# ubuntuslave/vo_single_camera_sos

Measured on AMD Instinct MI355X. Metric: frame-pairs/sec (detect+match+triangulate+RANSAC) on 640x480 omni, 2000 kpts, higher is better.
Workload: dtype u8/f32/f64

## Files before the change

include/sosvo.h:

```cpp
#ifndef SOSVO_H
#define SOSVO_H

#include <stdint.h>

#ifdef __cplusplus
extern "C" {
#endif

typedef struct sosvo_ctx sosvo_ctx;

typedef enum {
  SOSVO_OK = 0,
  SOSVO_ERR_ARG = -1,
  SOSVO_ERR_HIP = -2,
  SOSVO_ERR_NODEVICE = -3,
  SOSVO_ERR_CAPACITY = -4
} sosvo_status;

#define SOSVO_DESC_BYTES 32
#define SOSVO_KEY_SHIFT 20
#define SOSVO_KEY_IDX_MASK 0xFFFFFu
#define SOSVO_KEY_NONE 0xFFFFFFFFu


int32_t sosvo_abi_version(void);

int32_t sosvo_orb_bit_pattern_31(int8_t* pattern_host);

int32_t sosvo_create(sosvo_ctx** out, int32_t device, void* stream);
int32_t sosvo_destroy(sosvo_ctx* ctx);
int32_t sosvo_set_stream(sosvo_ctx* ctx, void* stream);
#define SOSVO_HINT_SHARED_DEVICE 1
#define SOSVO_HINT_SCORE_FP64_ONLY 2
int32_t sosvo_set_hint(sosvo_ctx* ctx, int32_t hint, int32_t value);
int32_t sosvo_synchronize(sosvo_ctx* ctx);
const char* sosvo_last_error(const sosvo_ctx* ctx);

int32_t sosvo_timer_start(sosvo_ctx* ctx);
int32_t sosvo_timer_stop(sosvo_ctx* ctx);
int32_t sosvo_timer_elapsed_ms(sosvo_ctx* ctx, float* ms);

int32_t sosvo_profile_enable(sosvo_ctx* ctx, int32_t on);
int32_t sosvo_profile_count(sosvo_ctx* ctx);
int32_t sosvo_profile_get(sosvo_ctx* ctx, int32_t i, char* name_out, int32_t name_cap, float* ms);

int32_t sosvo_debug_fill_scratch(sosvo_ctx* ctx, int32_t byte);

int32_t sosvo_unwrap(sosvo_ctx* ctx, const uint8_t* omni, const uint8_t* masks, const float* map_x,
                     const float* map_y, int32_t nframes, int32_t H, int32_t W, int32_t rows,
                     int32_t cols, uint8_t* pano);

int32_t sosvo_unwrap_prepare(sosvo_ctx* ctx, const uint8_t* masks, const float* map_x, const float* map_y,
                             int32_t H, int32_t W, int32_t rows, int32_t cols, uint32_t* table);
int32_t sosvo_unwrap_table(sosvo_ctx* ctx, const uint8_t* omni, const uint32_t* table, int32_t nframes,
                           int32_t H, int32_t W, int32_t rows, int32_t cols, uint8_t* pano);

int32_t sosvo_median_gray(sosvo_ctx* ctx, const uint8_t* img, int32_t nimg, int32_t rows,
                          int32_t cols, int32_t ksize, uint8_t* gray);
int32_t sosvo_unwrap_median_gray(sosvo_ctx* ctx, const uint8_t* omni, const uint32_t* table, int32_t nframes,
                                 int32_t H, int32_t W, int32_t rows, int32_t cols, int32_t ksize, uint8_t* gray);

int32_t sosvo_unwrap_median_gray_rows(sosvo_ctx* ctx, const uint8_t* omni, const uint32_t* table, int32_t nframes,
                                      int32_t H, int32_t W, int32_t rows, int32_t cols, int32_t ksize,
                                      const int32_t* row_range, uint8_t* gray);

int32_t sosvo_gray_rows_needed(sosvo_ctx* ctx, const uint32_t* mask_bits, int32_t nsets, int32_t rows, int32_t cols,
                               int32_t nmask, int32_t edge, const int8_t* pattern, float cos_a, float sin_a,
                               int32_t* row_range);

int32_t sosvo_detect_gft(sosvo_ctx* ctx, const uint8_t* gray, const uint32_t* mask_bits, int32_t nimg,
                         int32_t images_per_maskset, int32_t rows, int32_t cols, int32_t nmask,
                         double quality, double min_distance, int32_t max_corners, int32_t cap,
                         float* kp, int32_t* n, int32_t* status);

int32_t sosvo_describe_orb(sosvo_ctx* ctx, const uint8_t* gray, int32_t nimg, int32_t rows, int32_t cols,
                           int32_t nmask, int32_t cap, float* kp, int32_t* n, float cos_a, float sin_a,
                           const int8_t* pattern, int32_t edge, uint8_t* desc);

int32_t sosvo_describe_orb_rows(sosvo_ctx* ctx, const uint8_t* gray, int32_t nimg, int32_t rows, int32_t cols,
                                int32_t nmask, int32_t cap, float* kp, int32_t* n, float cos_a, float sin_a,
                                const int8_t* pattern, int32_t edge, const int32_t* row_range, uint8_t* desc);

int64_t sosvo_orb_pyramid_pixels(int32_t rows, int32_t cols);
int32_t sosvo_orb_mask_pyramid(sosvo_ctx* ctx, const uint32_t* mask_bits, int32_t nsets, int32_t rows,
                               int32_t cols, int32_t nmask, uint32_t* mask_pyr);
int32_t sosvo_detect_orb(sosvo_ctx* ctx, const uint8_t* gray, const uint32_t* mask_pyr, int32_t nimg,
                         int32_t images_per_maskset, int32_t rows, int32_t cols, int32_t nmask,
                         int32_t nfeatures, int32_t cap, float* kp4, float* resp, int32_t* n);
int32_t sosvo_describe_orb_levels(sosvo_ctx* ctx, const uint8_t* gray, int32_t nimg, int32_t rows,
                                  int32_t cols, int32_t nmask, int32_t cap, float* kp4, int32_t* n,
                                  const int8_t* pattern, uint8_t* desc, float* kp_xy);
int32_t sosvo_detect_describe_orb(sosvo_ctx* ctx, const uint8_t* gray, const uint32_t* mask_pyr, int32_t nimg,
                                  int32_t images_per_maskset, int32_t rows, int32_t cols, int32_t nmask,
                                  int32_t nfeatures, int32_t cap, float* kp4, float* resp, int32_t* n,
                                  const int8_t* pattern, uint8_t* desc, float* kp_xy);

int32_t sosvo_detect_fast(sosvo_ctx* ctx, const uint8_t* gray, const uint32_t* mask_bits, int32_t nimg,
                          int32_t images_per_maskset, int32_t rows, int32_t cols, int32_t nmask,
                          int32_t threshold, int32_t cap, float* kp, int32_t* n, int32_t* status);

int32_t sosvo_detect_agast(sosvo_ctx* ctx, const uint8_t* gray, const uint32_t* mask_bits, int32_t nimg,
                           int32_t images_per_maskset, int32_t rows, int32_t cols, int32_t nmask,
                           int32_t threshold, int32_t cap, float* kp, int32_t* n, int32_t* status);

int32_t sosvo_match_hamming(sosvo_ctx* ctx, const uint8_t* q_desc, const uint8_t* t_desc,
                            const int32_t* nq, const int32_t* nt, const int32_t* q_slot,
                            const int32_t* t_slot, int32_t nprob, int32_t q_stride,
                            int32_t t_stride, int32_t k, uint32_t* keys);

int32_t sosvo_match_hamming_gated(sosvo_ctx* ctx, const uint8_t* q_desc, const uint8_t* t_desc, const float* q_pos,
                                  const float* t_pos, const int32_t* nq, const int32_t* nt, const int32_t* q_slot,
                                  const int32_t* t_slot, int32_t nprob, int32_t n_forward, int32_t q_stride, int32_t t_stride,
                                  double min_dv, double max_du, int32_t max_distance, uint32_t* keys);

// ... 246 lines not shown
```

vo_single_camera_sos_amd/_lib.py:

```python
import ctypes
import os
import re

_HERE = os.path.dirname(os.path.abspath(__file__))
LIB_PATH = os.path.join(_HERE, "libsosvo.so")
HEADER_PATH = os.path.join(os.path.dirname(_HERE), "include", "sosvo.h")

c_i32 = ctypes.c_int32
c_f64 = ctypes.c_double
c_f32 = ctypes.c_float
c_u64 = ctypes.c_uint64
c_p = ctypes.c_void_p

SOSVO_OK = 0
STATUS_NAMES = {0: "SOSVO_OK", -1: "SOSVO_ERR_ARG", -2: "SOSVO_ERR_HIP", -3: "SOSVO_ERR_NODEVICE",
                -4: "SOSVO_ERR_CAPACITY"}

KEY_SHIFT = 20
KEY_IDX_MASK = 0xFFFFF
KEY_NONE = 0xFFFFFFFF
DESC_BYTES = 32


class SosvoError(RuntimeError):
    pass


SIGNATURES = {
    "sosvo_abi_version": (c_i32, []),
    "sosvo_orb_bit_pattern_31": (c_i32, [c_p]),
    "sosvo_create": (c_i32, [ctypes.POINTER(c_p), c_i32, c_p]),
    "sosvo_destroy": (c_i32, [c_p]),
    "sosvo_set_stream": (c_i32, [c_p, c_p]),
    "sosvo_set_hint": (c_i32, [c_p, c_i32, c_i32]),
    "sosvo_synchronize": (c_i32, [c_p]),
    "sosvo_last_error": (ctypes.c_char_p, [c_p]),
    "sosvo_timer_start": (c_i32, [c_p]),
    "sosvo_timer_stop": (c_i32, [c_p]),
    "sosvo_timer_elapsed_ms": (c_i32, [c_p, ctypes.POINTER(c_f32)]),
    "sosvo_profile_enable": (c_i32, [c_p, c_i32]),
    "sosvo_profile_count": (c_i32, [c_p]),
    "sosvo_debug_fill_scratch": (c_i32, [c_p, c_i32]),
    "sosvo_profile_get": (c_i32, [c_p, c_i32, ctypes.c_char_p, c_i32, ctypes.POINTER(c_f32)]),
    "sosvo_unwrap": (c_i32, [c_p, c_p, c_p, c_p, c_p, c_i32, c_i32, c_i32, c_i32, c_i32, c_p]),
    "sosvo_unwrap_prepare": (c_i32, [c_p, c_p, c_p, c_p, c_i32, c_i32, c_i32, c_i32, c_p]),
    "sosvo_unwrap_table": (c_i32, [c_p, c_p, c_p, c_i32, c_i32, c_i32, c_i32, c_i32, c_p]),
    "sosvo_median_gray": (c_i32, [c_p, c_p, c_i32, c_i32, c_i32, c_i32, c_p]),
    "sosvo_unwrap_median_gray": (c_i32, [c_p, c_p, c_p, c_i32, c_i32, c_i32, c_i32, c_i32, c_i32, c_p]),
    "sosvo_unwrap_median_gray_rows": (c_i32, [c_p, c_p, c_p, c_i32, c_i32, c_i32, c_i32, c_i32, c_i32, c_p, c_p]),
    "sosvo_gray_rows_needed": (c_i32, [c_p, c_p, c_i32, c_i32, c_i32, c_i32, c_i32, c_p, c_f32, c_f32, c_p]),
    "sosvo_detect_gft": (c_i32, [c_p, c_p, c_p, c_i32, c_i32, c_i32, c_i32, c_i32, c_f64, c_f64, c_i32, c_i32, c_p,
                                 c_p, c_p]),
    "sosvo_describe_orb": (c_i32, [c_p, c_p, c_i32, c_i32, c_i32, c_i32, c_i32, c_p, c_p, c_f32, c_f32, c_p, c_i32,
                                   c_p]),
    "sosvo_describe_orb_rows": (c_i32, [c_p, c_p, c_i32, c_i32, c_i32, c_i32, c_i32, c_p, c_p, c_f32, c_f32, c_p, c_i32,
                                        c_p, c_p]),
    "sosvo_orb_pyramid_pixels": (ctypes.c_int64, [c_i32, c_i32]),
    "sosvo_orb_mask_pyramid": (c_i32, [c_p, c_p, c_i32, c_i32, c_i32, c_i32, c_p]),
    "sosvo_detect_orb": (c_i32, [c_p, c_p, c_p, c_i32, c_i32, c_i32, c_i32, c_i32, c_i32, c_i32, c_p, c_p, c_p]),
    "sosvo_describe_orb_levels": (c_i32, [c_p, c_p, c_i32, c_i32, c_i32, c_i32, c_i32, c_p, c_p, c_p, c_p, c_p]),
    "sosvo_detect_describe_orb": (c_i32, [c_p, c_p, c_p, c_i32, c_i32, c_i32, c_i32, c_i32, c_i32, c_i32, c_p, c_p, c_p, c_p,
                                          c_p, c_p]),
    "sosvo_detect_fast": (c_i32, [c_p, c_p, c_p, c_i32, c_i32, c_i32, c_i32, c_i32, c_i32, c_i32, c_p, c_p, c_p]),
    "sosvo_detect_agast": (c_i32, [c_p, c_p, c_p, c_i32, c_i32, c_i32, c_i32, c_i32, c_i32, c_i32, c_p, c_p, c_p]),
    "sosvo_match_hamming": (c_i32, [c_p, c_p, c_p, c_p, c_p, c_p, c_p, c_i32, c_i32, c_i32, c_i32, c_p]),
    "sosvo_match_hamming_gated": (c_i32, [c_p, c_p, c_p, c_p, c_p, c_p, c_p, c_p, c_p, c_i32, c_i32, c_i32, c_i32, c_f64, c_f64,
                                          c_i32, c_p]),
    "sosvo_match_radius": (c_i32, [c_p, c_p, c_p, c_p, c_p, c_p, c_p, c_i32, c_i32, c_i32, c_i32, c_i32, c_p, c_p]),
    "sosvo_cross_check_matches": (c_i32, [c_p, c_p, c_p, c_p, c_p, c_p, c_p, c_i32, c_i32, c_i32, c_p, c_p]),
    "sosvo_sort_matches": (c_i32, [c_p, c_p, c_p, c_p, c_i32, c_i32, c_p]),
    "sosvo_pano_to_bearing": (c_i32, [c_p, c_p, c_i32, c_f64, c_f64, c_f64, c_f64, c_p, c_p, c_p]),
    "sosvo_triangulate_midpoint": (c_i32, [c_p, c_p, c_p, c_p, c_p, c_i32, c_p, c_p, c_p]),
    "sosvo_triangulate2": (c_i32, [c_p, c_p, c_p, c_i32, c_p, c_p, c_p]),
    "sosvo_range_filter": (c_i32, [c_p, c_p, c_i32, c_f64, c_f64, c_p]),
    "sosvo_rgbd_backproject": (c_i32, [c_p, c_p, c_i32, c_i32, c_p, c_p, c_i32, c_f64, c_f64, c_f64, c_f64, c_f64,
                                       c_i32, c_p, c_p]),
    "sosvo_stereo_assemble": (c_i32, [c_p] + [c_p] * 9 + [c_i32] * 4 + [c_p] * 9),
    "sosvo_f2f_assemble": (c_i32, [c_p] + [c_p] * 7 + [c_i32] + [c_p] * 6 + [c_i32, c_i32] + [c_p] * 7),
    "sosvo_ransac_abs_pose": (c_i32, [c_p, c_p, c_p, c_p, c_p, c_p, c_i32, c_i32, c_p, c_i32, c_i32, c_f64,
                                      c_i32, c_i32, c_u64, c_p, c_p, c_p, c_p, c_p, c_p]),
    "sosvo_ransac_abs_pose_seeds": (c_i32, [c_p, c_p, c_p, c_p, c_p, c_p, c_i32, c_i32, c_p, c_i32, c_i32, c_f64,
                                            c_i32, c_i32, c_p, c_p, c_p, c_p, c_p, c_p, c_p]),
    "sosvo_match_l2": (c_i32, [c_p, c_p, c_p, c_p, c_p, c_i32, c_i32, c_i32, c_i32, c_i32, c_p]),
    "sosvo_ransac_rel_pose": (c_i32, [c_p, c_p, c_p, c_p, c_i32, c_i32, c_i32, c_f64, c_i32, c_i32, c_u64, c_p, c_p, c_p, c_p,
                                      c_p, c_p]),
    "sosvo_refine_abs_pose": (c_i32, [c_p, c_p, c_p, c_p, c_p, c_p, c_i32, c_p, c_i32, c_i32, c_p, c_p, c_i32,
                                      c_p, c_p, c_p]),
    "sosvo_rgbd_assemble": (c_i32, [c_p, c_p, c_p, c_p, c_p, c_p, c_i32, c_i32, c_i32, c_i32, c_i32, c_p, c_p, c_p, c_p, c_p]),
    "sosvo_f2f_assemble_central": (c_i32, [c_p, c_f64, c_f64, c_p, c_p, c_p, c_p, c_i32, c_p, c_p, c_p, c_p, c_i32, c_i32,
                                           c_p, c_p, c_p, c_p, c_p]),
    "sosvo_frame_pair_batch_workspace": (ctypes.c_size_t, [c_p]),
    "sosvo_frame_pair_batch": (c_i32, [c_p, c_p, c_p, c_p, c_p, c_p, c_p, c_p, ctypes.c_size_t, c_p]),
    "sosvo_frame_pair_batch_streams_workspace": (ctypes.c_size_t, [c_p, c_i32]),
    "sosvo_frame_pair_batch_streams": (c_i32, [c_p, c_p, c_p, c_i32, c_p, c_p, c_p, c_p, c_p, ctypes.c_size_t, c_p]),
    "sosvo_frame_pair_batch_streams_enqueue": (c_i32, [c_p, c_p, c_p, c_i32, c_p, c_p, c_p, c_p, c_p, ctypes.c_size_t, c_p]),
    "sosvo_frame_pair_batch_streams_join": (c_i32, [c_p]),
    "sosvo_sequence_workspace": (ctypes.c_size_t, [c_p, c_i32, c_i32]),
    "sosvo_sequence_front_end": (c_i32, [c_p, c_p, c_p, c_i32, c_i32, c_p, c_i32, c_i32, c_p, c_p, c_p, c_p, ctypes.c_size_t]),
    "sosvo_sequence_track": (c_i32, [c_p, c_p, c_p, c_i32, c_i32, c_p, c_p, c_i32, c_u64, c_p, ctypes.c_size_t, c_p]),
    "sosvo_sequence_copy_slot": (c_i32, [c_p, c_p, c_i32, c_i32, c_i32, c_i32, c_p, ctypes.c_size_t]),
    "sosvo_sequence_frame_counts": (c_i32, [c_p, c_p, c_i32, c_i32, c_i32, c_i32, c_p, ctypes.c_size_t, c_p]),
    "sosvo_sequence_front_end_slots": (c_i32, [c_p, c_p, c_p, c_i32, c_i32, c_p, c_i32, c_p, c_p, c_p, c_p, c_p, ctypes.c_size_t]),
    "sosvo_sequence_track_seeds": (c_i32, [c_p, c_p, c_p, c_i32, c_i32, c_p, c_p, c_p, c_i32, c_p, ctypes.c_size_t, c_p]),
    "sosvo_sequence_copy_slots": (c_i32, [c_p, c_p, c_i32, c_i32, c_p, c_p, c_i32, c_p, ctypes.c_size_t]),
    "sosvo_rgbd_sequence_workspace": (ctypes.c_size_t, [c_p, c_i32, c_i32]),
    "sosvo_rgbd_sequence_front_end": (c_i32, [c_p, c_p, c_p, c_i32, c_i32, c_p, c_p, c_i32, c_i32, c_p, c_p, c_p, ctypes.c_size_t]),
    "sosvo_rgbd_sequence_track": (c_i32, [c_p, c_p, c_i32, c_i32, c_p, c_p, c_i32, c_u64, c_p, ctypes.c_size_t, c_p]),
    "sosvo_rgbd_sequence_copy_slot": (c_i32, [c_p, c_p, c_i32, c_i32, c_i32, c_i32, c_p, ctypes.c_size_t]),
    "sosvo_rgbd_sequence_frame_counts": (c_i32, [c_p, c_p, c_i32, c_i32, c_i32, c_i32, c_p, ctypes.c_size_t, c_p]),
    "sosvo_rgbd_sequence_front_end_slots": (c_i32, [c_p, c_p, c_p, c_i32, c_i32, c_p, c_p, c_i32, c_p, c_p, c_p, c_p,
                                                    ctypes.c_size_t]),
    "sosvo_rgbd_sequence_track_seeds": (c_i32, [c_p, c_p, c_i32, c_i32, c_p, c_p, c_p, c_i32, c_p, ctypes.c_size_t, c_p]),
    "sosvo_rgbd_sequence_copy_slots": (c_i32, [c_p, c_p, c_i32, c_i32, c_p, c_p, c_i32, c_p, ctypes.c_size_t]),
    "sosvo_rgbd_pair_batch_workspace": (ctypes.c_size_t, [c_p]),
    "sosvo_rgbd_pair_batch": (c_i32, [c_p, c_p, c_p, c_p, c_p, c_p, c_p, c_p, ctypes.c_size_t, c_p]),
}

HINT_SHARED_DEVICE = 1
HINT_SCORE_FP64_ONLY = 2
FLAG_CAM_ROT_IDENTITY = 1
FLAG_EPNP = 2
FLAG_GP3P = 4
FLAG_TWOPT = 8
FLAG_CROSS_CHECK_STEREO = 0x1000
FLAG_CROSS_CHECK_F2F = 0x2000
FLAG_GATED_STEREO = 0x4000
FLAG_GATED_F2F = 0x8000
GATED_MAX_DIST_SHIFT = 16
GATED_MAX_DIST_MASK = 0x1FF << GATED_MAX_DIST_SHIFT
DETECTOR_GFT = 0
DETECTOR_ORB = 1
DETECTOR_FAST = 2
DETECTOR_AGAST = 3
DETECTORS = {"GFT": DETECTOR_GFT, "ORB": DETECTOR_ORB, "FAST": DETECTOR_FAST, "AGAST": DETECTOR_AGAST}
RGBD_DETECTOR_SHIFT = 8
RGBD_DETECTOR_MASK = 3 << RGBD_DETECTOR_SHIFT
REL_FIVEPT = 5
REL_SEVENPT = 7
REL_EIGHTPT = 8


class Rig(ctypes.Structure):
    _fields_ = [("pano_top", c_f64 * 4), ("pano_bot", c_f64 * 4), ("F_top", c_f64 * 3), ("F_bot", c_f64 * 3),
                ("min_range", c_f64), ("max_range", c_f64), ("stereo_min_disp", c_f64),
                ("stereo_max_hdiff", c_f64), ("f2f_max_hdiff", c_f64), ("pct_good_matches", c_f64)]



class RgbdCam(ctypes.Structure):
    _fields_ = [("fx", c_f64), ("fy", c_f64), ("cx", c_f64), ("cy", c_f64), ("focal_length_m", c_f64),
                ("depth_is_Z", c_i32), ("reserved", c_i32), ("min_range", c_f64), ("max_range", c_f64)]

# ... 74 lines not shown
```

vo_single_camera_sos_amd/csrc/common.h:

```cpp
#pragma once
#include <hip/hip_runtime.h>
#include <stdint.h>
#include <stdio.h>
#include <string.h>

#include "sosvo.h"

struct sosvo_prof_entry {
  const char* name;
  hipEvent_t a, b;
};

constexpr int kSosvoProfMax = 16384;

constexpr int kSosvoMaxSubStreams = 4;

struct sosvo_ctx {
  int32_t device;
  hipStream_t stream;
  hipEvent_t ev_start, ev_stop;
  char err[512];
  void* ws;
  size_t ws_bytes;
  int32_t prof_on;
  int32_t prof_n;
  int32_t prof_created;
  sosvo_prof_entry* prof;
  sosvo_ctx* sub[kSosvoMaxSubStreams];
  hipEvent_t sub_done[kSosvoMaxSubStreams], sub_median[kSosvoMaxSubStreams], sub_begin;
  int32_t n_sub;
  int32_t hint_score_fp64_only;
  int32_t hint_shared_device;
  int32_t sub_last;
  int32_t sub_pending;
  const void* sub_last_ws;
  size_t sub_last_bytes[kSosvoMaxSubStreams];
};

struct SosvoProfScope {
  sosvo_ctx* ctx;
  bool active;
  SosvoProfScope(sosvo_ctx* c, const char* name) : ctx(c), active(false) {
    if (!c->prof_on || !c->prof || c->prof_n >= kSosvoProfMax) return;
    sosvo_prof_entry& e = c->prof[c->prof_n];
    if (c->prof_n >= c->prof_created) {
      if (hipEventCreate(&e.a) != hipSuccess || hipEventCreate(&e.b) != hipSuccess) return;
      c->prof_created = c->prof_n + 1;
    }
    e.name = name;
    if (hipEventRecord(e.a, c->stream) != hipSuccess) return;
    active = true;
  }
  ~SosvoProfScope() {
    if (!active) return;
    (void)hipEventRecord(ctx->prof[ctx->prof_n].b, ctx->stream);
    ctx->prof_n++;
  }
};
#define SOSVO_PROFILE(ctx, name) SosvoProfScope sosvo_prof_scope_(ctx, name)

#define SOSVO_LAUNCH(ctx, kernel, ...)            \
  do {                                            \
    SOSVO_PROFILE(ctx, #kernel);                  \
    hipLaunchKernelGGL(kernel, __VA_ARGS__);      \
// ... 106 lines not shown
```

vo_single_camera_sos_amd/csrc/ctx.hip:

```cpp
#include "common.h"
#include "orb_bit_pattern_31.h"

#include <stdlib.h>

extern "C" {

int32_t sosvo_abi_version(void) { return 1; }

int32_t sosvo_orb_bit_pattern_31(int8_t* pattern_host) {
  if (!pattern_host) return SOSVO_ERR_ARG;
  memcpy(pattern_host, sosvo_orb_bit_pattern_31_table, 1024);
  return SOSVO_OK;
}

int32_t sosvo_create(sosvo_ctx** out, int32_t device, void* stream) {
  if (!out) return SOSVO_ERR_ARG;
  *out = nullptr;
  int n = 0;
  if (hipGetDeviceCount(&n) != hipSuccess || n <= 0) return SOSVO_ERR_NODEVICE;
  if (device < 0 || device >= n) return SOSVO_ERR_NODEVICE;
  hipDeviceProp_t prop;
  if (hipGetDeviceProperties(&prop, device) != hipSuccess) return SOSVO_ERR_HIP;
  if (strncmp(prop.gcnArchName, "gfx950", 6) != 0) return SOSVO_ERR_NODEVICE;
  sosvo_ctx* ctx = (sosvo_ctx*)calloc(1, sizeof(sosvo_ctx));
  if (!ctx) return SOSVO_ERR_HIP;
  ctx->device = device;
  ctx->stream = (hipStream_t)stream;
  if (hipSetDevice(device) != hipSuccess || hipEventCreate(&ctx->ev_start) != hipSuccess ||
      hipEventCreate(&ctx->ev_stop) != hipSuccess) {
    free(ctx);
    return SOSVO_ERR_HIP;
  }
  *out = ctx;
  return SOSVO_OK;
}

int32_t sosvo_set_hint(sosvo_ctx* ctx, int32_t hint, int32_t value) {
  if (!ctx) return SOSVO_ERR_ARG;
  if (hint == SOSVO_HINT_SHARED_DEVICE) {
    ctx->hint_shared_device = value != 0;
  } else if (hint == SOSVO_HINT_SCORE_FP64_ONLY) {
    ctx->hint_score_fp64_only = value != 0;
    for (int i = 0; i < ctx->n_sub; ++i)
      if (ctx->sub[i]) ctx->sub[i]->hint_score_fp64_only = value != 0;
  } else {
    return sosvo_fail(ctx, SOSVO_ERR_ARG, __func__, "unknown hint");
  }
  return SOSVO_OK;
}

int32_t sosvo_destroy(sosvo_ctx* ctx) {
  if (!ctx) return SOSVO_OK;
  (void)hipSetDevice(ctx->device);
  for (int i = 0; i < ctx->n_sub; ++i) {
    if (ctx->sub[i]) {
      hipStream_t st = ctx->sub[i]->stream;
      (void)hipStreamSynchronize(st);
      (void)sosvo_destroy(ctx->sub[i]);
      (void)hipStreamDestroy(st);
    }
    (void)hipEventDestroy(ctx->sub_done[i]);
    (void)hipEventDestroy(ctx->sub_median[i]);
  }
  if (ctx->n_sub) (void)hipEventDestroy(ctx->sub_begin);
  if (ctx->ws) (void)hipFree(ctx->ws);
  if (ctx->prof) {
    for (int i = 0; i < ctx->prof_created; ++i) {
      (void)hipEventDestroy(ctx->prof[i].a);
      (void)hipEventDestroy(ctx->prof[i].b);
    }
    free(ctx->prof);
  }
  (void)hipEventDestroy(ctx->ev_start);
  (void)hipEventDestroy(ctx->ev_stop);
  free(ctx);
  return SOSVO_OK;
}
// ... 71 lines not shown
```

vo_single_camera_sos_amd/csrc/detect.hip:

```cpp
#include "common.h"

#include <type_traits>

namespace {

constexpr int kThreads = 256;
constexpr int kCandCap = 4096;
constexpr int kCandCapSmall = 2048;
constexpr int kCandCapLarge = 16384;
constexpr int kMaxMasks = 32;

__device__ __forceinline__ int refl101(int i, int n) {
  if (n == 1) return 0;
  while (i < 0 || i >= n) i = i < 0 ? -i : 2 * (n - 1) - i;
  return i;
}

__device__ __forceinline__ int clampi(int v, int lo, int hi) { return v < lo ? lo : (v > hi ? hi : v); }

__device__ __forceinline__ int lane_from_left(int v) { return __builtin_amdgcn_update_dpp(0, v, 0x138, 0xF, 0xF, true); }
__device__ __forceinline__ int lane_from_right(int v) { return __builtin_amdgcn_update_dpp(0, v, 0x130, 0xF, 0xF, true); }
__device__ __forceinline__ float lane_from_left(float v) { return __int_as_float(lane_from_left(__float_as_int(v))); }
__device__ __forceinline__ float lane_from_right(float v) { return __int_as_float(lane_from_right(__float_as_int(v))); }

// ... 679 lines not shown
    if (t > t_last) return;
    const int c = c_pre[P];
    int l1, l2, l3, r1, r2, r3;
    if (EDGE) {
      l3 = __shfl(c, src[0]); l2 = __shfl(c, src[1]); l1 = __shfl(c, src[2]);
      r1 = __shfl(c, src[4]); r2 = __shfl(c, src[5]); r3 = __shfl(c, src[6]);
    } else {
      l1 = lane_from_left(c); l2 = lane_from_left(l1); l3 = lane_from_left(l2);
      r1 = lane_from_right(c); r2 = lane_from_right(r1); r3 = lane_from_right(r2);
    }
    h[P] = mad24(18u, (uint32_t)(l3 + r3), mad24(34u, (uint32_t)(l2 + r2), mad24(49u, (uint32_t)(l1 + r1), 54u * (uint32_t)c)));
    const int y = t - 3;
    if (y < ys) return;
    const uint32_t vsum = mad24(18u, h[(P + 1) % 7] + h[P], mad24(34u, h[(P + 2) % 7] + h[(P + 6) % 7],
                                mad24(49u, h[(P + 3) % 7] + h[(P + 5) % 7], 54u * h[(P + 4) % 7])));
    if (out_lane) o[(uint32_t)(y * cols) + (uint32_t)xc] = (uint8_t)((vsum + 32768u) >> 16);
  };
  auto run = [&](auto edge_tag) __attribute__((always_inline)) {
    for (int t = t_first; t <= t_last; t += 7) {
      step(std::integral_constant<int, 0>{}, edge_tag, t);
      step(std::integral_constant<int, 1>{}, edge_tag, t + 1);
      step(std::integral_constant<int, 2>{}, edge_tag, t + 2);
      step(std::integral_constant<int, 3>{}, edge_tag, t + 3);
      request(t + 7, 0, 4);
      step(std::integral_constant<int, 4>{}, edge_tag, t + 4);
      step(std::integral_constant<int, 5>{}, edge_tag, t + 5);
      step(std::integral_constant<int, 6>{}, edge_tag, t + 6);
      request(t + 7, 4, 7);
    }
  };
  if (edge_strip) run(std::true_type{}); else run(std::false_type{});
}

constexpr int kPatchMaxR = 23, kPatchRows = 48, kPatchStride = 64;
constexpr int kDescRegionBytesGft = 24 * 1024;
typedef uint32_t __attribute__((aligned(1))) u32_unaligned;
template <int NT>
__global__ __launch_bounds__(NT) void orb_describe_kernel(const uint8_t* __restrict__ blurred, int rows, int cols,
                                                                int nmask, int cap, float* __restrict__ kp,
                                                                int32_t* __restrict__ n_io, float cos_a, float sin_a,
                                                                const int8_t* __restrict__ pattern, int edge,
                                                                uint8_t* __restrict__ desc, int nimg_total,
                                                                const int32_t* __restrict__ row_range, int imgs_per_range) {
  SOSVO_LATENCY_BOUND_PRIO();
  extern __shared__ float lds_kp[];
  __shared__ int off[512];
  __shared__ uint16_t poff[512];
  constexpr int kPatchWords = (NT / 64) * (kPatchRows * kPatchStride / 4);
  constexpr int kRegionWords = NT == 256 ? kDescRegionBytesGft / 4 : 0;
  __shared__ uint32_t patch_area[kPatchWords > kRegionWords ? kPatchWords : kRegionWords];
  __shared__ int wave_off[NT / 64 + 1];
  __shared__ int s_running, s_R;
  __shared__ int s_bb[4];
  const int tid = threadIdx.x, lane = tid & 63, wid = tid >> 6;
  const int p = xcd_problem(nimg_total, nmask);
  if (p < 0) return;
  const int img = p / nmask;
  const int n = min(n_io[p], cap);
  if (tid == 0) {
    s_running = 0;
    s_R = 0;
  }
  __syncthreads();
  for (int i = tid; i < 512; i += NT) {
    const float px = (float)pattern[2 * i], py = (float)pattern[2 * i + 1];
    const float xr = (px * cos_a) - (py * sin_a), yr = (px * sin_a) + (py * cos_a);
// ... 150 lines not shown
#pragma unroll
      for (int r = 0; r < 4; ++r) {
        const unsigned long long bal = __ballot(patch[pa[r]] < patch[pb[r]]);
        if (lane == r) mine = bal;
      }
      if (lane < 4) d[lane] = mine;
    }
    return;
  }
  for (int j = wid; j < m; j += NT / 64) {
    const uint8_t* c = im + (size_t)__float2int_rn(lds_kp[2 * j + 1]) * cols + __float2int_rn(lds_kp[2 * j]);
    unsigned long long* d = reinterpret_cast<unsigned long long*>(desc + ((size_t)p * cap + j) * 32);
#pragma unroll
    for (int r = 0; r < 4; ++r) {
      const int t = 64 * r + lane;
      const unsigned long long bal = __ballot(c[off[2 * t]] < c[off[2 * t + 1]]);
      if (lane == 0) d[r] = bal;
    }
  }
}

static void rolling_chunks(int nimg, int rows, int strips, int* nchunks, int* chunk_rows) {
  int nc = cdiv(16384, nimg * strips);
  if (nc > rows / 24) nc = rows / 24;
  if (nc < 1) nc = 1;
  *chunk_rows = cdiv(rows, nc);
  *nchunks = cdiv(rows, *chunk_rows);
}

}

static int32_t launch_gauss7_rows(sosvo_ctx* ctx, const uint8_t* in, long long in_stride, int nimg, int rows, int cols,
                                  uint8_t* out, long long out_stride, const int32_t* row_range, int imgs_per_range) {
  const int strips = cdiv(cols, kEigStripW);
  int nchunks, chunk_rows;
  rolling_chunks(nimg, rows, strips, &nchunks, &chunk_rows);
  SOSVO_LAUNCH(ctx, gauss7_kernel, dim3(cdiv(nimg * strips * nchunks, kThreads / 64)), dim3(kThreads), 0, ctx->stream, in,
               in_stride, nimg, rows, cols, strips, nchunks, chunk_rows, out, out_stride, row_range, imgs_per_range);
  SOSVO_LAUNCH_CHECK(ctx);
  return SOSVO_OK;
}
int32_t sosvo_launch_gauss7_rows(sosvo_ctx* ctx, const uint8_t* in, long long in_stride, int nimg, int rows, int cols,
                                 uint8_t* out, long long out_stride, const int32_t* row_range, int imgs_per_range) {
  return launch_gauss7_rows(ctx, in, in_stride, nimg, rows, cols, out, out_stride, row_range, imgs_per_range);
}
int32_t sosvo_launch_gauss7_to(sosvo_ctx* ctx, const uint8_t* in, long long in_stride, int nimg, int rows, int cols,
                               uint8_t* out, long long out_stride) {
  return launch_gauss7_rows(ctx, in, in_stride, nimg, rows, cols, out, out_stride, nullptr, 1);
}
int32_t sosvo_launch_gauss7(sosvo_ctx* ctx, const uint8_t* in, long long img_stride, int nimg, int rows, int cols,
                            uint8_t* out) {
  return sosvo_launch_gauss7_to(ctx, in, img_stride, nimg, rows, cols, out, img_stride);
}

extern "C" {

int32_t sosvo_detect_gft(sosvo_ctx* ctx, const uint8_t* gray, const uint32_t* mask_bits, int32_t nimg,
                         int32_t images_per_maskset, int32_t rows, int32_t cols, int32_t nmask, double quality,
                         double min_distance, int32_t max_corners, int32_t cap, float* kp, int32_t* n,
                         int32_t* status) {
  SOSVO_ENTER(ctx);
  SOSVO_REQUIRE(ctx, gray && mask_bits && kp && n, "null pointer");
  SOSVO_REQUIRE(ctx, nimg >= 0 && nimg <= 65535 && images_per_maskset > 0, "nimg out of range");
  SOSVO_REQUIRE(ctx, rows >= 3 && cols >= 3 && rows * (int64_t)cols < (1 << 28), "image sizes out of range");
  SOSVO_REQUIRE(ctx, nmask >= 1 && nmask <= kMaxMasks, "nmask out of range (1..32)");
  SOSVO_REQUIRE(ctx, cap > 0 && cap <= 4096 && quality > 0 && min_distance >= 0, "bad detector parameters (quality > 0)");
  if (nimg == 0) return SOSVO_OK;
  const size_t P = (size_t)nimg * nmask;
  size_t off = 0;
  auto carve = [&](size_t bytes) {
    size_t o = off;
    off += (bytes + 255) & ~(size_t)255;
    return o;
  };
  const int strips = cdiv(cols, kEigStripW);
  int nchunks, chunk_rows;
  rolling_chunks(nimg, rows, strips, &nchunks, &chunk_rows);
  const int wcap = (chunk_rows * kEigStripW + 63) & ~63;
  const size_t n_waves = (size_t)nimg * strips * nchunks;
  const size_t o_cand = carve(sizeof(uint2) * n_waves * wcap);
  const size_t o_wcnt = carve(sizeof(uint32_t) * n_waves);
  const size_t o_stat = carve(sizeof(uint32_t) * P * 5);
  const bool large = cap > 1024;
  const int sorted_stride = large ? kCandCapLarge : kCandCap;
  const size_t o_sorted = carve(sizeof(uint32_t) * P * sorted_stride);
  const size_t o_redo = carve(sizeof(int32_t) * P);
  int32_t rc = sosvo_ws_reserve(ctx, off);
  if (rc != SOSVO_OK) return rc;
// ... 85 lines not shown
```

vo_single_camera_sos_amd/csrc/pipeline.hip:

```cpp
#include <vector>

#include "common.h"

namespace {

struct Carver {
  char* base;
  size_t off = 0;
  template <typename T>
  T* take(size_t count) {
    T* p = base ? reinterpret_cast<T*>(base + off) : nullptr;
    off += (count * sizeof(T) + 255) & ~(size_t)255;
    return p;
  }
};

struct OrbBufs {
  float *kp4 = nullptr, *resp = nullptr;
  uint32_t* mask_pyr = nullptr;
};
OrbBufs carve_orb(Carver& cv, int detector, size_t P, size_t cap, size_t nsets, int rows, int cols) {
  OrbBufs o;
  if (detector != SOSVO_DETECTOR_ORB) return o;
  o.kp4 = cv.take<float>(P * cap * 4);
// ... 603 lines not shown
  for (int s = 0; s < n_streams; ++s) {
    int lo, hi;
    part_range(cfg->n_pairs, s, n_streams, &lo, &hi);
    sosvo_batch_cfg c = *cfg;
    c.n_pairs = hi - lo;
    const size_t bytes = sosvo_frame_pair_batch_workspace(&c);
    if (bytes == 0) return 0;
    total += (bytes + 255) & ~(size_t)255;
  }
  return total;
}

static int32_t sosvo_frame_pair_batch_streams_impl(sosvo_ctx* ctx, const sosvo_rig* rig, const sosvo_batch_cfg* cfg, int32_t n_streams,
                             const uint8_t* omni, const uint32_t* unwrap_table, const uint32_t* mask_bits,
                             const int8_t* pattern, void* workspace, size_t workspace_bytes, double* results, bool join) {
  SOSVO_REQUIRE(ctx, n_streams >= 1 && n_streams <= kSosvoMaxSubStreams, "n_streams out of range (1..4)");
  SOSVO_REQUIRE(ctx, cfg->n_pairs >= n_streams && cfg->n_pairs <= 8192, "n_pairs out of range (n_streams..8192)");
  SOSVO_REQUIRE(ctx, detector_ok(cfg->detector, cfg->kp_cap), "unknown detector, or ORB with kp_cap > 2048");
  SOSVO_REQUIRE(ctx, ((uintptr_t)workspace & 255) == 0, "workspace must be 256-byte aligned");
  const size_t need = sosvo_frame_pair_batch_streams_workspace(cfg, n_streams);
  SOSVO_REQUIRE(ctx, need > 0 && workspace_bytes >= need, "workspace too small (see sosvo_frame_pair_batch_streams_workspace)");
  while (ctx->n_sub < n_streams) {
    const int i = ctx->n_sub;
    if (i == 0) SOSVO_HIP(ctx, hipEventCreateWithFlags(&ctx->sub_begin, hipEventDisableTiming));
    hipStream_t st;
    SOSVO_HIP(ctx, hipStreamCreateWithFlags(&st, hipStreamNonBlocking));
    const int32_t rc = sosvo_create(&ctx->sub[i], ctx->device, st);
    if (rc != SOSVO_OK) {
      (void)hipStreamDestroy(st);
      return sosvo_fail(ctx, rc, __func__, "cannot create an internal stream context");
    }
    ctx->sub[i]->hint_shared_device = 1;
    ctx->sub[i]->hint_score_fp64_only = ctx->hint_score_fp64_only;
    SOSVO_HIP(ctx, hipEventCreateWithFlags(&ctx->sub_done[i], hipEventDisableTiming));
    SOSVO_HIP(ctx, hipEventCreateWithFlags(&ctx->sub_median[i], hipEventDisableTiming));
    ctx->n_sub = i + 1;
  }
  size_t bytes[kSosvoMaxSubStreams];
  for (int s = 0; s < n_streams; ++s) {
    int lo, hi;
    part_range(cfg->n_pairs, s, n_streams, &lo, &hi);
    sosvo_batch_cfg c = *cfg;
    c.n_pairs = hi - lo;
    bytes[s] = (sosvo_frame_pair_batch_workspace(&c) + 255) & ~(size_t)255;
  }
  if (ctx->sub_pending) {
    hipStreamCaptureStatus cap = hipStreamCaptureStatusNone;
    SOSVO_HIP(ctx, hipStreamIsCapturing(ctx->stream, &cap));
    SOSVO_REQUIRE(ctx, cap == hipStreamCaptureStatusNone,
                  "un-joined sosvo_frame_pair_batch_streams_enqueue work is pending: call ..._join before capturing");
    bool same = ctx->sub_last == n_streams && ctx->sub_last_ws == workspace;
    for (int s = 0; same && s < n_streams; ++s) same = ctx->sub_last_bytes[s] == bytes[s];
    if (!same) {
      for (int s = 0; s < ctx->sub_last; ++s) SOSVO_HIP(ctx, hipStreamWaitEvent(ctx->stream, ctx->sub_done[s], 0));
      ctx->sub_pending = 0;
    }
  }
  SOSVO_HIP(ctx, hipEventRecord(ctx->sub_begin, ctx->stream));
  char* ws = reinterpret_cast<char*>(workspace);
  hipEvent_t token = (ctx->sub_pending && ctx->sub_last > 0) ? ctx->sub_median[ctx->sub_last - 1] : nullptr;
  for (int s = 0; s < n_streams; ++s) {
    int lo, hi;
    part_range(cfg->n_pairs, s, n_streams, &lo, &hi);
    sosvo_batch_cfg c = *cfg;
    c.n_pairs = hi - lo;
    c.seed = cfg->seed + (uint64_t)lo;
// ... 448 lines not shown
```

vo_single_camera_sos_amd/device.py:

```python
import ctypes

import torch

from . import _lib
from ._lib import SosvoError, c_f32, c_p

NULL = c_p(0)


def _ptr(t):
    return c_p(t.data_ptr()) if t is not None else NULL


def _check(t, dtype, name, shape=None, ndim=None):
    if not isinstance(t, torch.Tensor):
        raise SosvoError("%s: expected a torch tensor, got %r" % (name, type(t)))
    if not t.is_cuda:
        raise SosvoError("%s: must live on the GPU" % name)
    if t.dtype != dtype:
        raise SosvoError("%s: dtype %s, expected %s" % (name, t.dtype, dtype))
    if not t.is_contiguous():
        raise SosvoError("%s: must be contiguous" % name)
    if ndim is not None and t.dim() != ndim:
        raise SosvoError("%s: ndim %d, expected %d" % (name, t.dim(), ndim))
# ... 28 lines not shown
        torch.cuda.set_device(self.device)
        if stream is None:
            stream = torch.cuda.current_stream(self.device)
        self.stream = stream
        h = c_p()
        rc = self._lib.sosvo_create(ctypes.byref(h), int(device), c_p(stream.cuda_stream))
        if rc != 0:
            raise SosvoError("sosvo_create failed: %s" % _lib.STATUS_NAMES.get(rc, rc))
        self._h = h

    def close(self):
        if getattr(self, "_h", None) is not None:
            self._lib.sosvo_destroy(self._h)
            self._h = None

    def __del__(self):
        try:
            self.close()
        except Exception:
            pass

    def _call(self, fn, *args):
        rc = fn(self._h, *args)
        if rc != 0:
            msg = self._lib.sosvo_last_error(self._h)
            raise SosvoError("%s -> %s: %s" % (fn.__name__, _lib.STATUS_NAMES.get(rc, rc),
                                               msg.decode() if msg else ""))

    def set_hint_shared_device(self, on=True):
        self._call(self._lib.sosvo_set_hint, _lib.HINT_SHARED_DEVICE, 1 if on else 0)

    def set_hint_score_fp64_only(self, on=True):
        self._call(self._lib.sosvo_set_hint, _lib.HINT_SCORE_FP64_ONLY, 1 if on else 0)

    def set_stream(self, stream):
        self._call(self._lib.sosvo_set_stream, c_p(stream.cuda_stream))
        self.stream = stream

    def synchronize(self):
        self._call(self._lib.sosvo_synchronize)

    def timer_start(self):
        self._call(self._lib.sosvo_timer_start)

    def timer_stop(self):
        self._call(self._lib.sosvo_timer_stop)

    def timer_elapsed_ms(self):
        ms = c_f32()
        self._call(self._lib.sosvo_timer_elapsed_ms, ctypes.byref(ms))
        return float(ms.value)

    def debug_fill_scratch(self, byte=0xFF):
        self._call(self._lib.sosvo_debug_fill_scratch, int(byte))

    def profile_enable(self, on=True):
        self._call(self._lib.sosvo_profile_enable, 1 if on else 0)

    def profile_read(self):
        n = self._lib.sosvo_profile_count(self._h)
        buf = ctypes.create_string_buffer(128)
        ms = c_f32()
        out = []
        for i in range(n):
            self._call(self._lib.sosvo_profile_get, i, buf, 128, ctypes.byref(ms))
            out.append((buf.value.decode(), float(ms.value)))
# ... 106 lines not shown
            raise SosvoError("mask_bits has too few sets for %d images" % NI)
        P = NI * nmask
        dev = gray.device
        if kp is None:
            kp = torch.zeros((P, cap, 2), dtype=torch.float32, device=dev)
        if n is None:
            n = torch.zeros((P,), dtype=torch.int32, device=dev)
        if status is None:
            status = torch.zeros((P,), dtype=torch.int32, device=dev)
        _check(kp, torch.float32, "kp", (P, cap, 2))
        _check(n, torch.int32, "n", (P,))
        _check(status, torch.int32, "status", (P,))
        self._call(self._lib.sosvo_detect_gft, _ptr(gray), _ptr(mask_bits), NI, int(images_per_maskset), rows, cols,
                   int(nmask), float(quality), float(min_distance), int(max_corners), int(cap), _ptr(kp), _ptr(n),
                   _ptr(status))
        return kp, n, status

    def describe_orb(self, gray, kp, n, nmask, pattern, cos_a, sin_a, edge=31, desc=None, row_range=None):
        _check(gray, torch.uint8, "gray", ndim=3)
        NI, rows, cols = gray.shape
        P = NI * nmask
        _check(kp, torch.float32, "kp", (P, None, 2))
        cap = kp.shape[1]
        _check(n, torch.int32, "n", (P,))
        _check(pattern, torch.int8, "pattern", (512, 2))
        if desc is None:
            desc = torch.zeros((P, cap, 32), dtype=torch.uint8, device=gray.device)
        _check(desc, torch.uint8, "desc", (P, cap, 32))
        if row_range is not None:
            _check(row_range, torch.int32, "row_range", (2, 2))
        self._call(self._lib.sosvo_describe_orb_rows, _ptr(gray), NI, rows, cols, int(nmask), cap, _ptr(kp), _ptr(n),
                   float(cos_a), float(sin_a), _ptr(pattern), int(edge), _ptr(row_range), _ptr(desc))
        return desc

    def orb_pyramid_pixels(self, rows, cols):
        return int(self._lib.sosvo_orb_pyramid_pixels(int(rows), int(cols)))

    def orb_mask_pyramid(self, mask_bits, nmask):
        _check(mask_bits, torch.uint32, "mask_bits", ndim=3)
        nsets, rows, cols = mask_bits.shape
        out = torch.zeros((nsets, self.orb_pyramid_pixels(rows, cols)), dtype=torch.uint32, device=mask_bits.device)
        self._call(self._lib.sosvo_orb_mask_pyramid, _ptr(mask_bits), nsets, rows, cols, int(nmask), _ptr(out))
        return out

    def detect_orb(self, gray, mask_pyr, images_per_maskset, nmask, nfeatures, cap, kp4=None, resp=None, n=None):
        _check(gray, torch.uint8, "gray", ndim=3)
        NI, rows, cols = gray.shape
        _check(mask_pyr, torch.uint32, "mask_pyr", (None, self.orb_pyramid_pixels(rows, cols)))
        if mask_pyr.shape[0] * images_per_maskset < NI:
            raise SosvoError("mask_pyr has too few sets for %d images" % NI)
        P = NI * nmask
        dev = gray.device
        if kp4 is None:
            kp4 = torch.zeros((P, cap, 4), dtype=torch.float32, device=dev)
        if resp is None:
            resp = torch.zeros((P, cap), dtype=torch.float32, device=dev)
        if n is None:
            n = torch.zeros((P,), dtype=torch.int32, device=dev)
        _check(kp4, torch.float32, "kp4", (P, cap, 4))
        _check(resp, torch.float32, "resp", (P, cap))
        _check(n, torch.int32, "n", (P,))
        self._call(self._lib.sosvo_detect_orb, _ptr(gray), _ptr(mask_pyr), NI, int(images_per_maskset), rows, cols,
                   int(nmask), int(nfeatures), int(cap), _ptr(kp4), _ptr(resp), _ptr(n))
        return kp4, resp, n

    def describe_orb_levels(self, gray, kp4, n, nmask, pattern, desc=None, kp_xy=None):
# ... 610 lines not shown
```

Baseline: 63330.

## Compute 7-tap Gaussian blur with int8 MFMA banded-matrix products

Adds a gauss7 kernel that does the separable 7-tap Gaussian as two int8 32x32x32 MFMA matrix products against banded tap matrices. The horizontal result is split into high and low bytes with a bias correction, and reflective borders are folded into the band matrices. It becomes the default path for images of at least 32x32, with a hint to fall back to the old VALU kernel, and it also exposes a standalone gauss7 API. The aim is to cut the ALU cost of the blur stage, at the price of exact-rounding complexity and some redundant overlap loads.

Result: no change. 63210 (-0.2%).

```diff
diff --git a/include/sosvo.h b/include/sosvo.h
--- a/include/sosvo.h
+++ b/include/sosvo.h
@@ -32,6 +32,7 @@
 int32_t sosvo_set_stream(sosvo_ctx* ctx, void* stream);
 #define SOSVO_HINT_SHARED_DEVICE 1
 #define SOSVO_HINT_SCORE_FP64_ONLY 2
+#define SOSVO_HINT_GAUSS7_VALU 3
 int32_t sosvo_set_hint(sosvo_ctx* ctx, int32_t hint, int32_t value);
 int32_t sosvo_synchronize(sosvo_ctx* ctx);
 const char* sosvo_last_error(const sosvo_ctx* ctx);
@@ -80,6 +81,9 @@
 int32_t sosvo_describe_orb_rows(sosvo_ctx* ctx, const uint8_t* gray, int32_t nimg, int32_t rows, int32_t cols,
                                 int32_t nmask, int32_t cap, float* kp, int32_t* n, float cos_a, float sin_a,
                                 const int8_t* pattern, int32_t edge, const int32_t* row_range, uint8_t* desc);
+
+int32_t sosvo_gauss7_rows(sosvo_ctx* ctx, const uint8_t* gray, int64_t in_stride, int32_t nimg, int32_t rows, int32_t cols,
+                          uint8_t* out, int64_t out_stride, const int32_t* row_range, int32_t imgs_per_range);
 
 int64_t sosvo_orb_pyramid_pixels(int32_t rows, int32_t cols);
 int32_t sosvo_orb_mask_pyramid(sosvo_ctx* ctx, const uint32_t* mask_bits, int32_t nsets, int32_t rows,
diff --git a/vo_single_camera_sos_amd/_lib.py b/vo_single_camera_sos_amd/_lib.py
--- a/vo_single_camera_sos_amd/_lib.py
+++ b/vo_single_camera_sos_amd/_lib.py
@@ -55,6 +55,7 @@
                                    c_p]),
     "sosvo_describe_orb_rows": (c_i32, [c_p, c_p, c_i32, c_i32, c_i32, c_i32, c_i32, c_p, c_p, c_f32, c_f32, c_p, c_i32,
                                         c_p, c_p]),
+    "sosvo_gauss7_rows": (c_i32, [c_p, c_p, ctypes.c_int64, c_i32, c_i32, c_i32, c_p, ctypes.c_int64, c_p, c_i32]),
     "sosvo_orb_pyramid_pixels": (ctypes.c_int64, [c_i32, c_i32]),
     "sosvo_orb_mask_pyramid": (c_i32, [c_p, c_p, c_i32, c_i32, c_i32, c_i32, c_p]),
     "sosvo_detect_orb": (c_i32, [c_p, c_p, c_p, c_i32, c_i32, c_i32, c_i32, c_i32, c_i32, c_i32, c_p, c_p, c_p]),
@@ -118,6 +119,7 @@
 
 HINT_SHARED_DEVICE = 1
 HINT_SCORE_FP64_ONLY = 2
+HINT_GAUSS7_VALU = 3
 FLAG_CAM_ROT_IDENTITY = 1
 FLAG_EPNP = 2
 FLAG_GP3P = 4
diff --git a/vo_single_camera_sos_amd/csrc/common.h b/vo_single_camera_sos_amd/csrc/common.h
--- a/vo_single_camera_sos_amd/csrc/common.h
+++ b/vo_single_camera_sos_amd/csrc/common.h
@@ -30,6 +30,7 @@
   hipEvent_t sub_done[kSosvoMaxSubStreams], sub_median[kSosvoMaxSubStreams], sub_begin;
   int32_t n_sub;
   int32_t hint_score_fp64_only;
+  int32_t hint_gauss7_valu;
   int32_t hint_shared_device;
   int32_t sub_last;
   int32_t sub_pending;
diff --git a/vo_single_camera_sos_amd/csrc/ctx.hip b/vo_single_camera_sos_amd/csrc/ctx.hip
--- a/vo_single_camera_sos_amd/csrc/ctx.hip
+++ b/vo_single_camera_sos_amd/csrc/ctx.hip
@@ -43,6 +43,10 @@
     ctx->hint_score_fp64_only = value != 0;
     for (int i = 0; i < ctx->n_sub; ++i)
       if (ctx->sub[i]) ctx->sub[i]->hint_score_fp64_only = value != 0;
+  } else if (hint == SOSVO_HINT_GAUSS7_VALU) {
+    ctx->hint_gauss7_valu = value != 0;
+    for (int i = 0; i < ctx->n_sub; ++i)
+      if (ctx->sub[i]) ctx->sub[i]->hint_gauss7_valu = value != 0;
   } else {
     return sosvo_fail(ctx, SOSVO_ERR_ARG, __func__, "unknown hint");
   }
diff --git a/vo_single_camera_sos_amd/csrc/detect.hip b/vo_single_camera_sos_amd/csrc/detect.hip
--- a/vo_single_camera_sos_amd/csrc/detect.hip
+++ b/vo_single_camera_sos_amd/csrc/detect.hip
@@ -735,6 +735,103 @@
   if (edge_strip) run(std::true_type{}); else run(std::false_type{});
 }
 
+constexpr int kG7Out = 26;
+constexpr unsigned long long kG7Taps = 0x0012223136312212ULL;
+typedef int g7v4 __attribute__((ext_vector_type(4)));
+typedef int g7v16 __attribute__((ext_vector_type(16)));
+typedef g7v4 __attribute__((aligned(1))) g7v4_unaligned;
+
+template <bool PERM>
+__device__ __forceinline__ g7v4 g7_band_inner(int n, int half) {
+  g7v4 b;
+#pragma unroll
+  for (int q = 0; q < 4; ++q) {
+    const int off = (PERM ? 8 * q + 4 * half : 16 * half + 4 * q) - n;
+    const uint32_t v = off >= 0 ? (uint32_t)(kG7Taps >> (8 * min(off, 7))) : (uint32_t)(kG7Taps << (8 * min(-off, 4)));
+    b[q] = n < kG7Out ? (int)v : 0;
+  }
+  return b;
+}
+template <bool PERM>
+__device__ __forceinline__ g7v4 g7_band_border(int n, int half, int o0, int w0, int size, int nvalid) {
+  uint32_t b[4] = {0u, 0u, 0u, 0u};
+#pragma unroll
+  for (int d = 0; d < 7; ++d) {
+    int s = o0 + n + d - 3;
+    s = s < 0 ? -s : s;
+    s = s >= size ? 2 * (size - 1) - s : s;
+    const int k = s - w0;
+    const int khalf = PERM ? (k >> 2) & 1 : k >> 4, kq = PERM ? k >> 3 : (k >> 2) & 3;
+    const uint32_t w = (uint32_t)((kG7Taps >> (8 * d)) & 0xFFu) << (8 * (k & 3));
+#pragma unroll
+    for (int q = 0; q < 4; ++q) b[q] += (n < nvalid && khalf == half && kq == q) ? w : 0u;
+  }
+  return g7v4{(int)b[0], (int)b[1], (int)b[2], (int)b[3]};
+}
+
+__global__ __launch_bounds__(kThreads) void gauss7_mfma_kernel(const uint8_t* __restrict__ gray, long long img_stride, int nimg,
+                                                               int rows, int cols, int strips, int nchunks, int chunk_tiles,
+                                                               uint8_t* __restrict__ out, long long out_stride,
+                                                               const int32_t* __restrict__ row_range, int imgs_per_range) {
+  SOSVO_STREAMING_PRIO();
+  const int lane = threadIdx.x & 63, col = lane & 31, half = lane >> 5;
+  const int wave = __builtin_amdgcn_readfirstlane((int)((blockIdx.x * kThreads + threadIdx.x) >> 6));
+  if (wave >= nimg * strips * nchunks) return;
+  const int img = wave / (strips * nchunks);
+  const int rem = wave - img * strips * nchunks;
+  const int chunk = rem / strips, strip = rem - chunk * strips;
+  int ys = 0, ye = rows;
+  if (row_range) {
+    const int v = img / imgs_per_range;
+    ys = max(ys, row_range[2 * v]);
+    ye = min(ye, row_range[2 * v + 1]);
+  }
+  const int x0 = strip * kG7Out, nx = min(kG7Out, cols - x0);
+  const int wx = clampi(x0 - 3, 0, cols - 32);
+  const g7v4 bh = wx == x0 - 3 ? g7_band_inner<false>(col, half) : g7_band_border<false>(col, half, x0, wx, cols, nx);
+  const g7v4 av_inner = g7_band_inner<true>(col, half);
+  const uint8_t* g = gray + (size_t)img * img_stride + (uint32_t)(col * cols + wx + 16 * half);
+  uint8_t* o = out + (size_t)img * out_stride + (uint32_t)x0;
+  uint32_t o_lane[16];
+#pragma unroll
+  for (int r = 0; r < 16; ++r) o_lane[r] = (uint32_t)((8 * (r >> 2) + 4 * half + (r & 3)) * cols + col);
+  const g7v16 zero = {0, 0, 0, 0, 0, 0, 0, 0, 0, 0, 0, 0, 0, 0, 0, 0};
+  g7v4 c43 = {0x2B2B2B2B, 0x2B2B2B2B, 0x2B2B2B2B, 0x2B2B2B2B};
+  g7v4 c24 = {0x18181818, 0x18181818, 0x18181818, 0x18181818};
+  int y0 = ys + chunk * chunk_tiles * kG7Out;
+  if (y0 >= ye) return;
+  g7v4 a_next = *reinterpret_cast<const g7v4_unaligned*>(g + (uint32_t)(clampi(y0 - 3, 0, rows - 32) * cols));
+  for (int t = 0; t < chunk_tiles && y0 < ye; ++t, y0 += kG7Out) {
+    const int ny = min(kG7Out, ye - y0);
+    const int wy = clampi(y0 - 3, 0, rows - 32);
+    g7v4 av = av_inner;
+    if (wy != y0 - 3) av = g7_band_border<true>(col, half, y0, wy, rows, ny);
+    const g7v4 a = a_next ^ (int)0x80808080u;
+    a_next = *reinterpret_cast<const g7v4_unaligned*>(g + (uint32_t)(clampi(y0 + kG7Out - 3, 0, rows - 32) * cols));
+    const g7v16 h = __builtin_amdgcn_mfma_i32_32x32x32_i8(a, bh, zero, 0, 0, 0);
+    asm volatile("" : "+v"(c43), "+v"(c24));
+    const g7v16 c_hi = __builtin_amdgcn_mfma_i32_32x32x32_i8(c43, c24, zero, 0, 0, 0);
+    g7v4 b_hi, b_lo;
+#pragma unroll
+    for (int q = 0; q < 4; ++q) {
+      const uint32_t p01 = __builtin_amdgcn_perm((uint32_t)h[4 * q + 1], (uint32_t)h[4 * q + 0], 0x05010400u);
+      const uint32_t p23 = __builtin_amdgcn_perm((uint32_t)h[4 * q + 3], (uint32_t)h[4 * q + 2], 0x05010400u);
+      b_lo[q] = (int)(__builtin_amdgcn_perm(p23, p01, 0x05040100u) ^ 0x80808080u);
+      b_hi[q] = (int)__builtin_amdgcn_perm(p23, p01, 0x07060302u);
+    }
+    const g7v16 d_hi = __builtin_amdgcn_mfma_i32_32x32x32_i8(av, b_hi, c_hi, 0, 0, 0);
+    const g7v16 d_lo = __builtin_amdgcn_mfma_i32_32x32x32_i8(av, b_lo, zero, 0, 0, 0);
+    const int lim = col < nx ? ny - 4 * half : 0;
+    uint8_t* otile = o + (size_t)(uint32_t)(y0 * cols);
+#pragma unroll
+    for (int r = 0; r < 16; ++r) {
+      const uint32_t v = ((uint32_t)d_hi[r] << 8) + (uint32_t)d_lo[r];
+      asm volatile("" : "+v"(o_lane[r]));
+      if (8 * (r >> 2) + (r & 3) < lim) otile[o_lane[r]] = (uint8_t)(v >> 16);
+    }
+  }
+}
+
 constexpr int kPatchMaxR = 23, kPatchRows = 48, kPatchStride = 64;
 constexpr int kDescRegionBytesGft = 24 * 1024;
 typedef uint32_t __attribute__((aligned(1))) u32_unaligned;
@@ -951,6 +1048,19 @@
 
 static int32_t launch_gauss7_rows(sosvo_ctx* ctx, const uint8_t* in, long long in_stride, int nimg, int rows, int cols,
                                   uint8_t* out, long long out_stride, const int32_t* row_range, int imgs_per_range) {
+  if (rows >= 32 && cols >= 32 && !ctx->hint_gauss7_valu) {
+    const int strips = cdiv(cols, kG7Out), tiles = cdiv(rows, kG7Out);
+    int nc = cdiv(16384, nimg * strips);
+    nc = nc > tiles ? tiles : nc;
+    const int chunk_tiles = cdiv(tiles, nc), nchunks = cdiv(tiles, chunk_tiles);
+    {
+      SOSVO_PROFILE(ctx, "gauss7_kernel");
+      hipLaunchKernelGGL(gauss7_mfma_kernel, dim3(cdiv(nimg * strips * nchunks, kThreads / 64)), dim3(kThreads), 0, ctx->stream, in,
+                         in_stride, nimg, rows, cols, strips, nchunks, chunk_tiles, out, out_stride, row_range, imgs_per_range);
+    }
+    SOSVO_LAUNCH_CHECK(ctx);
+    return SOSVO_OK;
+  }
   const int strips = cdiv(cols, kEigStripW);
   int nchunks, chunk_rows;
   rolling_chunks(nimg, rows, strips, &nchunks, &chunk_rows);
@@ -973,6 +1083,18 @@
 }
 
 extern "C" {
+
+int32_t sosvo_gauss7_rows(sosvo_ctx* ctx, const uint8_t* gray, int64_t in_stride, int32_t nimg, int32_t rows, int32_t cols,
+                          uint8_t* out, int64_t out_stride, const int32_t* row_range, int32_t imgs_per_range) {
+  SOSVO_ENTER(ctx);
+  SOSVO_REQUIRE(ctx, gray && out, "null pointer");
+  SOSVO_REQUIRE(ctx, nimg >= 0 && nimg <= 65535, "nimg out of range");
+  SOSVO_REQUIRE(ctx, rows >= 1 && cols >= 1 && rows * (int64_t)cols < (1 << 28), "image sizes out of range");
+  SOSVO_REQUIRE(ctx, in_stride >= rows * (int64_t)cols && out_stride >= rows * (int64_t)cols, "images overlap (stride < rows * cols)");
+  SOSVO_REQUIRE(ctx, row_range == nullptr || imgs_per_range >= 1, "imgs_per_range must be positive");
+  if (nimg == 0) return SOSVO_OK;
+  return launch_gauss7_rows(ctx, gray, in_stride, nimg, rows, cols, out, out_stride, row_range, row_range ? imgs_per_range : 1);
+}
 
 int32_t sosvo_detect_gft(sosvo_ctx* ctx, const uint8_t* gray, const uint32_t* mask_bits, int32_t nimg,
                          int32_t images_per_maskset, int32_t rows, int32_t cols, int32_t nmask, double quality,
diff --git a/vo_single_camera_sos_amd/csrc/pipeline.hip b/vo_single_camera_sos_amd/csrc/pipeline.hip
--- a/vo_single_camera_sos_amd/csrc/pipeline.hip
+++ b/vo_single_camera_sos_amd/csrc/pipeline.hip
@@ -659,6 +659,7 @@
     }
     ctx->sub[i]->hint_shared_device = 1;
     ctx->sub[i]->hint_score_fp64_only = ctx->hint_score_fp64_only;
+    ctx->sub[i]->hint_gauss7_valu = ctx->hint_gauss7_valu;
     SOSVO_HIP(ctx, hipEventCreateWithFlags(&ctx->sub_done[i], hipEventDisableTiming));
     SOSVO_HIP(ctx, hipEventCreateWithFlags(&ctx->sub_median[i], hipEventDisableTiming));
     ctx->n_sub = i + 1;
diff --git a/vo_single_camera_sos_amd/device.py b/vo_single_camera_sos_amd/device.py
--- a/vo_single_camera_sos_amd/device.py
+++ b/vo_single_camera_sos_amd/device.py
@@ -84,6 +84,9 @@
 
     def set_hint_score_fp64_only(self, on=True):
         self._call(self._lib.sosvo_set_hint, _lib.HINT_SCORE_FP64_ONLY, 1 if on else 0)
+
+    def set_hint_gauss7_valu(self, on=True):
+        self._call(self._lib.sosvo_set_hint, _lib.HINT_GAUSS7_VALU, 1 if on else 0)
 
     def set_stream(self, stream):
         self._call(self._lib.sosvo_set_stream, c_p(stream.cuda_stream))
@@ -256,6 +259,40 @@
         self._call(self._lib.sosvo_describe_orb_rows, _ptr(gray), NI, rows, cols, int(nmask), cap, _ptr(kp), _ptr(n),
                    float(cos_a), float(sin_a), _ptr(pattern), int(edge), _ptr(row_range), _ptr(desc))
         return desc
+
+    def gauss7(self, gray, row_range=None, out=None, shape=None, in_stride=None, out_stride=None):
+        if shape is None:
+            _check(gray, torch.uint8, "gray", ndim=3)
+            NI, rows, cols = gray.shape
+        else:
+            _check(gray, torch.uint8, "gray", ndim=1)
+            NI, rows, cols = (int(v) for v in shape)
+        if NI < 0 or rows < 1 or cols < 1:
+            raise SosvoError("gauss7: bad shape %r" % ((NI, rows, cols),))
+        in_stride = rows * cols if in_stride is None else int(in_stride)
+        if out is None:
+            out_stride = rows * cols if out_stride is None else int(out_stride)
+            out = torch.zeros((NI, rows, cols) if shape is None and out_stride == rows * cols else
+                              (max(NI - 1, 0) * out_stride + rows * cols,), dtype=torch.uint8, device=gray.device)
+        else:
+            _check(out, torch.uint8, "out")
+            out_stride = rows * cols if out_stride is None else int(out_stride)
+        for name, t, stride in (("gray", gray, in_stride), ("out", out, out_stride)):
+            if stride < rows * cols:
+                raise SosvoError("gauss7: %s stride %d < rows * cols" % (name, stride))
+            if NI and t.numel() < (NI - 1) * stride + rows * cols:
+                raise SosvoError("gauss7: %s holds %d bytes, %d images of %d x %d at stride %d need more"
+                                 % (name, t.numel(), NI, rows, cols, stride))
+        per = 1
+        if row_range is not None:
+            _check(row_range, torch.int32, "row_range", (None, 2))
+            R = row_range.shape[0]
+            if R < 1 or NI % R:
+                raise SosvoError("gauss7: %d images do not split evenly over %d row ranges" % (NI, R))
+            per = max(NI // R, 1)
+        self._call(self._lib.sosvo_gauss7_rows, _ptr(gray), in_stride, NI, rows, cols, _ptr(out), out_stride, _ptr(row_range),
+                   per)
+        return out
 
     def orb_pyramid_pixels(self, rows, cols):
         return int(self._lib.sosvo_orb_pyramid_pixels(int(rows), int(cols)))
```
